# mmammel8/kmer_id

Hardware: AMD Instinct MI355X
Metric: paired reads classified/sec on bact10 DB (higher is better)
Workload: dtype u64

## Files before the change

### include/kmer_id_amd.h

```cpp
#ifndef KMER_ID_AMD_H
#define KMER_ID_AMD_H

#include <stddef.h>
#include <stdint.h>

#ifdef __cplusplus
extern "C" {
#endif

typedef enum kid_status {
    KID_OK = 0,
    KID_ERR_ARG = -1,
    KID_ERR_NOMEM = -2,
    KID_ERR_HIP = -3,
    KID_ERR_TABLE_FULL = -4,
    KID_ERR_TREE = -5,
    KID_ERR_NO_DEVICE = -6,
    KID_ERR_TARGET = -7,
    KID_ERR_IO = -8,
    KID_ERR_FORMAT = -9,
    KID_ERR_STATE = -10
} kid_status;

#define KID_FLAG_U_IS_T 1u
// ... 92 lines not shown
int kid_db_read_hits_time(kid_db *db, double *device_ms, uint64_t *calls, uint64_t *reads);

typedef struct kid_support {
    uint32_t final, confident, n_kmers, n_hits , s_final ,
        s_confident ;
} kid_support;
int kid_db_read_support(kid_db *db, const uint8_t *bases, const uint64_t *offsets, const int32_t *start, const int32_t *stop,
                        uint64_t n_reads, uint32_t min_hits, uint32_t min_permille, kid_support *out, kid_sample *tally);
int kid_db_read_support_fastq(kid_db *db, const uint8_t *text, uint64_t text_nbytes, const kid_fastq_rec *recs, uint64_t n_reads,
                              uint32_t min_hits, uint32_t min_permille, kid_support *out, kid_sample *tally);
int kid_db_support_from_hits_device(kid_db *db, const void *d_hit_offsets, const void *d_hits, const void *d_n_kmers, uint64_t n_reads,
                                    uint32_t min_hits, uint32_t min_permille, void *d_out, void *stream);
int kid_db_read_support_time(kid_db *db, double *device_ms, uint64_t *calls, uint64_t *reads);

#define KID_SEGMENT_MAX_OVERLAP 1024u
typedef struct kid_segment {
    uint32_t pos, n_pos, final, confident, n_kmers, n_hits, s_final, s_confident;
} kid_segment;
int kid_db_read_segments(kid_db *db, const uint8_t *bases, const uint64_t *offsets, const int32_t *start, const int32_t *stop,
                         uint64_t n_reads, uint32_t seg_len, uint32_t seg_step, uint32_t min_hits, uint32_t min_permille,
                         uint64_t *seg_offsets, kid_segment *segments, uint64_t cap, uint64_t *n_segments);
int kid_db_read_segments_fastq(kid_db *db, const uint8_t *text, uint64_t text_nbytes, const kid_fastq_rec *recs, uint64_t n_reads,
                               uint32_t seg_len, uint32_t seg_step, uint32_t min_hits, uint32_t min_permille, uint64_t *seg_offsets,
                               kid_segment *segments, uint64_t cap, uint64_t *n_segments);
int kid_db_read_segments_device(kid_db *db, const void *d_bases, uint64_t bases_nbytes, const void *d_offsets, const void *d_start,
                                const void *d_stop, uint64_t n_reads, uint32_t seg_len, uint32_t seg_step, uint32_t min_hits,
                                uint32_t min_permille, void *d_hits, uint64_t hits_cap, void *d_seg_offsets, void *d_segments,
                                uint64_t seg_cap, void *d_n_hits, void *d_n_segments, void *stream);
int kid_db_read_segments_time(kid_db *db, double *device_ms, uint64_t *calls, uint64_t *reads);

int kid_sample_end(kid_sample *s, int64_t *gcount, int64_t *ucount);
int kid_sample_end_merged(kid_sample **samples, int n, int64_t *gcount, int64_t *ucount);
int kid_sample_stats(kid_sample *s, uint64_t out[4]);

int kid_sample_set_timing(kid_sample *s, int enabled);
int kid_sample_kernel_time(kid_sample *s, double *total_ms, uint64_t *launches);
int kid_sample_kernel_time_device(kid_sample *s, double *total_ms, uint64_t *launches);

int kid_sample_seen_bytes(const kid_sample *s, uint64_t *nbytes);
int kid_sample_seen_export(kid_sample *s, uint64_t byte_off, uint64_t nbytes, void *dst, int dst_on_device);
int kid_sample_seen_or(kid_sample *s, uint64_t byte_off, uint64_t nbytes, const void *src, int src_on_device);
int kid_sample_gcount(kid_sample *s, int64_t *gcount);
int kid_sample_ucount_range(kid_sample *s, uint64_t bit_begin, uint64_t bit_end, int64_t *ucount);

int kid_sample_depth_export(kid_sample *s, uint64_t entry_begin, uint64_t n, void *dst, int dst_on_device);
int kid_sample_depth_add(kid_sample *s, uint64_t entry_begin, uint64_t n, const void *src, int src_on_device);
int kid_sample_depth_spectrum(kid_sample *s, uint32_t bins, uint64_t *spectrum, uint64_t *ksum, uint32_t *dmax);
int kid_sample_depth_spectrum_merged(kid_sample **samples, int n, uint32_t bins, uint64_t *spectrum, uint64_t *ksum, uint32_t *dmax);

typedef struct kid_builder kid_builder;
typedef struct kid_build_cand {
    uint64_t key;
    int64_t gpos;
    int32_t target;
    uint16_t count;
    uint8_t strand_r;
    uint8_t flags;
} kid_build_cand;
int kid_device_mem_info(int device, uint64_t *free_bytes, uint64_t *total_bytes);
int kid_builder_create(int device, int log2_cells, const int32_t *parent, int32_t ntar, uint64_t batch_bases, kid_builder **out);
void kid_builder_destroy(kid_builder *b);
int kid_builder_add(kid_builder *b, const uint8_t *text, uint64_t len, int32_t target);
int kid_builder_remove(kid_builder *b, const uint8_t *text, uint64_t len);
int kid_builder_set_minct(kid_builder *b, const int32_t *minct, int32_t n);
int kid_builder_claim(kid_builder *b, const uint8_t *text, uint64_t len, int64_t gpos_base, kid_build_cand *out, uint64_t cap,
                      uint64_t *n_out);
// ... 11 lines not shown
```

### kmer_id_amd/_lib.py

```python
import ctypes as C
import os

from . import _build

c_u8p = C.POINTER(C.c_uint8)
c_u32p = C.POINTER(C.c_uint32)
c_i32p = C.POINTER(C.c_int32)
c_u64p = C.POINTER(C.c_uint64)
c_i64p = C.POINTER(C.c_int64)
c_void_pp = C.POINTER(C.c_void_p)


class KidDbInfo(C.Structure):
    _fields_ = [
        ("ntar", C.c_int32), ("k", C.c_int32), ("log2_slots", C.c_int32), ("max_probes", C.c_int32),
        ("flags", C.c_uint32), ("device", C.c_int32), ("tree_depth", C.c_int32), ("host_built", C.c_int32),
        ("geometry", C.c_int32), ("reserved_", C.c_int32),
        ("n_entries", C.c_uint64), ("n_occupied", C.c_uint64), ("table_bytes", C.c_uint64),
    ]


PROTOTYPES = {
    "kid_strerror": (C.c_char_p, [C.c_int]),
    "kid_last_error": (C.c_char_p, []),
# ... 23 lines not shown
    "kid_classify_batch_device": (C.c_int, [C.c_void_p, C.c_void_p, C.c_uint64, C.c_void_p, C.c_void_p, C.c_void_p, C.c_uint64,
                                            C.c_void_p, C.c_void_p]),
    "kid_classify_fixed_device": (C.c_int, [C.c_void_p, C.c_void_p, C.c_uint32, C.c_uint64, C.c_void_p, C.c_void_p]),
    "kid_trim_batch": (C.c_int, [C.c_void_p, C.c_void_p, C.c_void_p, C.c_uint64, C.c_void_p, C.c_void_p, C.c_void_p]),
    "kid_db_set_option": (C.c_int, [C.c_void_p, C.c_int, C.c_int]),
    "kid_sample_masked_bases": (C.c_int, [C.c_void_p, c_u64p]),
    "kid_mask_batch": (C.c_int, [C.c_void_p, C.c_void_p, C.c_void_p, C.c_void_p, C.c_uint64, C.c_int, C.c_void_p, c_u64p]),
    "kid_mask_batch_device": (C.c_int, [C.c_void_p, C.c_void_p, C.c_void_p, C.c_void_p, C.c_uint64, C.c_int, C.c_void_p, C.c_void_p]),
    "kid_db_read_hits": (C.c_int, [C.c_void_p, C.c_void_p, C.c_void_p, C.c_void_p, C.c_void_p, C.c_uint64, C.c_void_p, C.c_void_p,
                                   C.c_void_p, C.c_uint64, c_u64p]),
    "kid_db_read_hits_fastq": (C.c_int, [C.c_void_p, C.c_void_p, C.c_uint64, C.c_void_p, C.c_uint64, C.c_void_p, C.c_void_p,
                                         C.c_void_p, C.c_uint64, c_u64p]),
    "kid_db_read_hits_device": (C.c_int, [C.c_void_p, C.c_void_p, C.c_uint64, C.c_void_p, C.c_void_p, C.c_void_p, C.c_uint64,
                                          C.c_void_p, C.c_void_p, C.c_void_p, C.c_uint64, C.c_void_p, C.c_void_p]),
    "kid_db_read_hits_time": (C.c_int, [C.c_void_p, C.POINTER(C.c_double), c_u64p, c_u64p]),
    "kid_db_read_support": (C.c_int, [C.c_void_p, C.c_void_p, C.c_void_p, C.c_void_p, C.c_void_p, C.c_uint64, C.c_uint32, C.c_uint32,
                                      C.c_void_p, C.c_void_p]),
    "kid_db_read_support_fastq": (C.c_int, [C.c_void_p, C.c_void_p, C.c_uint64, C.c_void_p, C.c_uint64, C.c_uint32, C.c_uint32,
                                            C.c_void_p, C.c_void_p]),
    "kid_db_support_from_hits_device": (C.c_int, [C.c_void_p, C.c_void_p, C.c_void_p, C.c_void_p, C.c_uint64, C.c_uint32, C.c_uint32,
                                                  C.c_void_p, C.c_void_p]),
    "kid_db_read_support_time": (C.c_int, [C.c_void_p, C.POINTER(C.c_double), c_u64p, c_u64p]),
    "kid_db_read_segments": (C.c_int, [C.c_void_p, C.c_void_p, C.c_void_p, C.c_void_p, C.c_void_p, C.c_uint64, C.c_uint32, C.c_uint32,
                                       C.c_uint32, C.c_uint32, C.c_void_p, C.c_void_p, C.c_uint64, c_u64p]),
    "kid_db_read_segments_fastq": (C.c_int, [C.c_void_p, C.c_void_p, C.c_uint64, C.c_void_p, C.c_uint64, C.c_uint32, C.c_uint32,
                                             C.c_uint32, C.c_uint32, C.c_void_p, C.c_void_p, C.c_uint64, c_u64p]),
    "kid_db_read_segments_device": (C.c_int, [C.c_void_p, C.c_void_p, C.c_uint64, C.c_void_p, C.c_void_p, C.c_void_p, C.c_uint64,
                                              C.c_uint32, C.c_uint32, C.c_uint32, C.c_uint32, C.c_void_p, C.c_uint64, C.c_void_p,
                                              C.c_void_p, C.c_uint64, C.c_void_p, C.c_void_p, C.c_void_p]),
    "kid_db_read_segments_time": (C.c_int, [C.c_void_p, C.POINTER(C.c_double), c_u64p, c_u64p]),
    "kid_sample_end": (C.c_int, [C.c_void_p, C.c_void_p, C.c_void_p]),
    "kid_sample_end_merged": (C.c_int, [c_void_pp, C.c_int, C.c_void_p, C.c_void_p]),
    "kid_sample_stats": (C.c_int, [C.c_void_p, C.c_void_p]),
    "kid_sample_set_timing": (C.c_int, [C.c_void_p, C.c_int]),
    "kid_sample_kernel_time": (C.c_int, [C.c_void_p, C.POINTER(C.c_double), c_u64p]),
    "kid_sample_kernel_time_device": (C.c_int, [C.c_void_p, C.POINTER(C.c_double), c_u64p]),
    "kid_sample_seen_bytes": (C.c_int, [C.c_void_p, c_u64p]),
    "kid_sample_seen_export": (C.c_int, [C.c_void_p, C.c_uint64, C.c_uint64, C.c_void_p, C.c_int]),
    "kid_sample_seen_or": (C.c_int, [C.c_void_p, C.c_uint64, C.c_uint64, C.c_void_p, C.c_int]),
    "kid_sample_gcount": (C.c_int, [C.c_void_p, C.c_void_p]),
    "kid_sample_ucount_range": (C.c_int, [C.c_void_p, C.c_uint64, C.c_uint64, C.c_void_p]),
    "kid_sample_depth_export": (C.c_int, [C.c_void_p, C.c_uint64, C.c_uint64, C.c_void_p, C.c_int]),
    "kid_sample_depth_add": (C.c_int, [C.c_void_p, C.c_uint64, C.c_uint64, C.c_void_p, C.c_int]),
    "kid_sample_depth_spectrum": (C.c_int, [C.c_void_p, C.c_uint32, C.c_void_p, C.c_void_p, C.c_void_p]),
    "kid_sample_depth_spectrum_merged": (C.c_int, [c_void_pp, C.c_int, C.c_uint32, C.c_void_p, C.c_void_p, C.c_void_p]),
    "kid_synth_db_keys_host": (C.c_int, [C.c_uint64, C.c_int, C.c_void_p, C.c_int32, C.c_uint64, C.c_uint64, C.c_void_p,
                                         C.c_void_p]),
    "kid_synth_db_keys_device": (C.c_int, [C.c_uint64, C.c_int, C.c_void_p, C.c_int32, C.c_uint64, C.c_uint64, C.c_void_p,
                                           C.c_void_p, C.c_int]),
    "kid_synth_reads_host": (C.c_int, [C.c_uint64, C.c_uint64, C.c_int, C.c_void_p, C.c_void_p, C.c_int32, C.c_uint64,
                                       C.c_uint64, C.c_uint32, C.c_void_p]),
    "kid_synth_reads_device": (C.c_int, [C.c_uint64, C.c_uint64, C.c_int, C.c_void_p, C.c_void_p, C.c_int32, C.c_uint64,
                                         C.c_uint64, C.c_uint32, C.c_void_p, C.c_int]),
    "kid_sample_kernel_variants": (C.c_int, [C.c_void_p, c_u64p]),
    "kid_bench_gather": (C.c_int, [C.c_void_p, C.c_uint64, C.c_int, C.c_int, C.POINTER(C.c_float), c_u64p]),
    "kid_dev_alloc": (C.c_int, [C.c_int, C.c_uint64, c_void_pp]),
    "kid_dev_free": (C.c_int, [C.c_int, C.c_void_p]),
    "kid_dev_upload": (C.c_int, [C.c_int, C.c_void_p, C.c_void_p, C.c_uint64]),
    "kid_dev_download": (C.c_int, [C.c_int, C.c_void_p, C.c_void_p, C.c_uint64]),
    "kid_dev_sync": (C.c_int, [C.c_int]),
    "kid_device_mem_info": (C.c_int, [C.c_int, c_u64p, c_u64p]),
    "kid_builder_create": (C.c_int, [C.c_int, C.c_int, C.c_void_p, C.c_int32, C.c_uint64, c_void_pp]),
    "kid_builder_destroy": (None, [C.c_void_p]),
    "kid_builder_add": (C.c_int, [C.c_void_p, C.c_void_p, C.c_uint64, C.c_int32]),
    "kid_builder_remove": (C.c_int, [C.c_void_p, C.c_void_p, C.c_uint64]),
    "kid_builder_set_minct": (C.c_int, [C.c_void_p, C.c_void_p, C.c_int32]),
# ... 64 lines not shown
```

### kmer_id_amd/api.py

```python
import ctypes as C

import numpy as np

from . import _lib
from ._lib import KidDbInfo, check


def _ptr(a):
    return a.ctypes.data_as(C.c_void_p) if a is not None else None


def _as(a, dtype):
    if a is None:
        return None
    a = np.ascontiguousarray(a, dtype=dtype)
    return a


def _offsets_batch(bases, offsets, start, stop):
    offsets = _as(offsets, np.uint64)
    return _as(bases, np.uint8), offsets, _as(start, np.int32), _as(stop, np.int32), offsets.size - 1


def _fastq_block(text, recs):
# ... 351 lines not shown
    def wait(self, ticket):
        check(self._lib.kid_classify_wait(self._h, ticket))

    def classify_device(self, d_bases, bases_nbytes, d_offsets, n_reads, d_start=0, d_stop=0, d_out=0, stream=0):
        check(self._lib.kid_classify_batch_device(self._h, C.c_void_p(d_bases), bases_nbytes, C.c_void_p(d_offsets),
                                                  C.c_void_p(d_start or None), C.c_void_p(d_stop or None), n_reads,
                                                  C.c_void_p(d_out or None), C.c_void_p(stream or None)))

    def classify_fixed_device(self, d_bases, read_len, n_reads, d_out=0, stream=0):
        check(self._lib.kid_classify_fixed_device(self._h, C.c_void_p(d_bases), read_len, n_reads,
                                                  C.c_void_p(d_out or None), C.c_void_p(stream or None)))

    def end(self):
        g = np.empty(self.ntar, np.int64)
        u = np.empty(self.ntar, np.int64)
        check(self._lib.kid_sample_end(self._h, _ptr(g), _ptr(u)))
        return g, u

    def gcount(self):
        g = np.empty(self.ntar, np.int64)
        check(self._lib.kid_sample_gcount(self._h, _ptr(g)))
        return g

    def ucount_range(self, slot_begin, slot_end):
        u = np.empty(self.ntar, np.int64)
        check(self._lib.kid_sample_ucount_range(self._h, slot_begin, slot_end, _ptr(u)))
        return u

    def stats(self):
        out = np.zeros(4, np.uint64)
        check(self._lib.kid_sample_stats(self._h, _ptr(out)))
        return {"reads": int(out[0]), "lookups": int(out[1]), "probes": int(out[2]), "hits": int(out[3])}

    def set_timing(self, enabled=True):
        check(self._lib.kid_sample_set_timing(self._h, 1 if enabled else 0))

    def kernel_time(self):
        ms, n = C.c_double(0), C.c_uint64(0)
        check(self._lib.kid_sample_kernel_time(self._h, C.byref(ms), C.byref(n)))
        return ms.value, n.value

    def kernel_time_device(self):
        ms, n = C.c_double(0), C.c_uint64(0)
        check(self._lib.kid_sample_kernel_time_device(self._h, C.byref(ms), C.byref(n)))
        return ms.value, n.value

    def kernel_variants(self):
        m = C.c_uint64(0)
        check(self._lib.kid_sample_kernel_variants(self._h, C.byref(m)))
        return {(b >> 3 & 1, b >> 2 & 1, b >> 1 & 1, 30 if b & 1 else 0, b >> 4) for b in range(64) if m.value >> b & 1}

    def seen_bytes(self):
        n = C.c_uint64(0)
        check(self._lib.kid_sample_seen_bytes(self._h, C.byref(n)))
        return n.value

    def seen_export(self, byte_off, nbytes, dst_ptr=None, on_device=False):
        if dst_ptr is None:
            buf = np.empty(nbytes, np.uint8)
            check(self._lib.kid_sample_seen_export(self._h, byte_off, nbytes, _ptr(buf), 0))
            return buf
        check(self._lib.kid_sample_seen_export(self._h, byte_off, nbytes, C.c_void_p(dst_ptr), 1 if on_device else 0))
        return None

    def seen_or(self, byte_off, src, nbytes=None, on_device=False):
        if isinstance(src, np.ndarray):
# ... 32 lines not shown
```

### kmer_id_amd/csrc/kid_api.hip

```cpp
#include <hip/hip_runtime.h>
#include <memory>
#include <stdint.h>
#include <string.h>
#include <type_traits>
#include <utility>
#include <vector>

#include "../../include/kmer_id_amd.h"
#include "kid_kernels.hip.h"
#include "kid_build.hip.h"
#include "kid_tile.hip.h"
#include "kid_long.hip.h"
#include "kid_hits.hip.h"
#include "kid_support.hip.h"
#include "kid_segments.hip.h"
#include "kid_mask.hip.h"
#include "kid_depth.hip.h"
#include "kid_api_core.h"
#include "kid_api_db.h"
#include "kid_api_mask.h"
#include "kid_api_hits.h"
#include "kid_api_builder.h"
#include "kid_api_bench.h"

// ... 11 lines not shown
    std::vector<std::pair<KidEvent, KidEvent>> timed;
    uint64_t timed_batches = 0;
    uint32_t batch_seq = 0;
    struct Scratch {
        KidDevBuf desc;
        KidDevBuf long_list;
        KidDevBuf long_plan;
        KidDevBuf rare;
        KidEvent ev_prep;
        KidEvent ev_used;
        hipStream_t used_stream = nullptr;
        bool used_recorded = false;
        bool used = false;
    };
    static const int NSET = 3;
    Scratch sets[NSET];
    uint32_t next_set = 0;
    bool inputs_ready = false;
    int min_base_quality = 0;
    KidDevBuf masked;
    int64_t long_kmers = 65536;
    KidDevBuf rare_fixed;
    struct { uint32_t *out_final = nullptr; uint64_t read0 = 0; uint32_t fixed_len = 0; int32_t fixed_nk = 0; bool valid = false; } fixed_held;
    uint64_t dev_clock_batches = 0;
    KidDevBuf seen_log, seen_log_tail, seen_sorted, log_counts, log_bin_total;
    uint32_t seen_log_cap = 0, log_nbins = 0;
    KidMappedHost log_host_total;
    bool log_dirty = false;
    bool log_off = false;
    uint32_t passes_done = 0;
    uint32_t launches_since_apply = 0;
    uint64_t reads_since_apply = 0;
    double log_entries_per_read = 4.0;
    uint64_t reads_of_last_pass = 0;
    KidDevBuf long_hits, long_tiles;
    bool ended = false;
    uint64_t reads_submitted = 0;
    uint64_t kernel_variants = 0;
    hipStream_t last_stream = nullptr;
    bool has_last_stream = false;
    KidEvent order_ev;
    struct Slot {
        KidDevBuf bases;
        KidDevBuf offsets, start, stop, out;
        KidDevBuf recs;
        KidEvent ev_h2d, ev_done, ev_out;
        std::vector<uint64_t> rel;
        uint64_t ticket = 0;
        bool busy = false;
    };
    static const int NSLOT = 3;
    Slot slots[NSLOT];
    uint64_t next_ticket = 1;

    unsigned long long *stats_p() const { return stats.as<unsigned long long>(); }
    volatile unsigned long long *log_rate() const { return static_cast<volatile unsigned long long *>(log_host_total.p); }
    volatile unsigned int *log_off_flag() const { return reinterpret_cast<volatile unsigned int *>(static_cast<char *>(log_host_total.p) + 8); }
};

extern "C" void kid_sample_destroy(kid_sample *s)
{
    if (!s) return;
    if (s->db) hipSetDevice(s->db->device);
    hipDeviceSynchronize();
    delete s;
}

static int kid_seenlog_point(kid_sample *s, hipStream_t stream);
extern "C" int kid_sample_reset(kid_sample *s)
{
    if (!s) return kid_fail(KID_ERR_ARG, "null sample");
    int rc = kid_use_device(s->db->device);
    if (rc != KID_OK) return rc;
    KID_HIP(hipDeviceSynchronize());
    const size_t nt = (size_t)s->db->info.ntar;
    KID_HIP(hipMemset(s->gcount.p, 0, nt * 8));
    KID_HIP(hipMemset(s->ucount.p, 0, nt * 8));
    KID_HIP(hipMemset(s->stats.p, 0, 256));
    KID_HIP(hipMemset(s->masked.p, 0, 8));
    {
        const unsigned long long never = ~0ull;
        KID_HIP(hipMemcpy(s->stats_p() + 30, &never, 8, hipMemcpyHostToDevice));
    }
    s->dev_clock_batches = 0;
    s->reads_submitted = 0;
    s->ended = false;
    s->kernel_variants = 0;
    if (s->seen_log_tail.p) KID_HIP(hipMemset(s->seen_log_tail.p, 0, KID_LOG_SHARDS * 64));
    if (s->seen_log.p) {
        int rc = kid_seenlog_point(s, nullptr);
        if (rc != KID_OK) return rc;
        *s->log_off_flag() = 0;
        *s->log_rate() = 0;
        s->log_off = false;
        s->passes_done = 0;
        s->log_entries_per_read = 4.0;
    }
    s->log_dirty = false;
    s->launches_since_apply = 0;
    s->reads_since_apply = 0;
    KID_HIP(hipMemset(s->seen.p, 0, s->seen_words * 4));
    if (s->depth.p) KID_HIP(hipMemset(s->depth.p, 0, s->seen_words * 32 * 4));
    KID_HIP(hipDeviceSynchronize());
    return KID_OK;
}

extern "C" int kid_sample_begin(kid_db *db, kid_sample **out)
{
    if (!db || !out) return kid_fail(KID_ERR_ARG, "null argument");
    *out = nullptr;
    int rc = kid_use_device(db->device);
    if (rc != KID_OK) return rc;
    std::unique_ptr<kid_sample, void (*)(kid_sample *)> s(new kid_sample(), kid_sample_destroy);
    s->db = db;
    const size_t nt = (size_t)db->info.ntar;
    s->seen_words = db->seen_bits / 32;
    KID_HIP(s->gcount.alloc(nt * 8));
    KID_HIP(s->ucount.alloc(nt * 8));
    KID_HIP(s->stats.alloc(256));
    KID_HIP(s->masked.alloc(8));
    KID_HIP(s->seen.alloc(s->seen_words * 4));
    KID_HIP(s->stream.create());
    const uint64_t nbins = (db->seen_bits + (1ull << KID_LOG_BIN_BITS) - 1) >> KID_LOG_BIN_BITS;
    if (db->d.minloc && nbins <= 1024) {
        uint64_t total = db->info.n_entries * 2ull;
        if (total < (32ull << 20)) total = 32ull << 20;
        if (total > (128ull << 20)) total = 128ull << 20;
        uint64_t cap = (total / KID_LOG_SHARDS) & ~63ull;
        s->seen_log_cap = (uint32_t)cap;
// ... 3 lines not shown
        KID_HIP(s->seen_log_tail.alloc(KID_LOG_SHARDS * 64));
        KID_HIP(s->log_counts.alloc(nbins * KID_LOG_WGS * 4));
        KID_HIP(s->log_bin_total.alloc(nbins * 4));
        KID_HIP(s->log_host_total.alloc(64, hipHostMallocMapped));
        memset(s->log_host_total.p, 0, 64);
    }
    const KidRareArgs ra{s->gcount.as<unsigned long long>(), s->stats_p(), db->d.line_mask, 0u, 0ull, 0ull, 0, 0u, db->d.rows,
                         s->seen.as<uint32_t>(), nullptr, nullptr, s->seen_log.as<uint32_t>(), s->seen_log_tail.as<uint32_t>(),
                         s->seen_log_cap, 0u};
    for (kid_sample::Scratch &sc : s->sets) {
        KID_HIP(sc.rare.alloc(sizeof(ra)));
        KID_HIP(hipMemcpy(sc.rare.p, &ra, sizeof(ra), hipMemcpyHostToDevice));
        KID_HIP(sc.ev_prep.create(hipEventDisableTiming));
        KID_HIP(sc.ev_used.create(hipEventDisableTiming));
    }
    KID_HIP(s->rare_fixed.alloc(sizeof(ra)));
    KID_HIP(hipMemcpy(s->rare_fixed.p, &ra, sizeof(ra), hipMemcpyHostToDevice));
    rc = kid_sample_reset(s.get());
    if (rc != KID_OK) return rc;
    *out = s.release();
    return KID_OK;
}

static int kid_seenlog_apply(kid_sample *s, hipStream_t stream)
{
    if (!s->seen_log.p || !s->log_dirty) return KID_OK;
    void *dev_total = nullptr;
    KID_HIP(hipHostGetDevicePointer(&dev_total, s->log_host_total.p, 0));
    const KidLogArgs a{s->seen_log.as<uint32_t>(), s->seen_log_tail.as<uint32_t>(), s->seen_log_cap, s->log_nbins,
                       s->log_counts.as<uint32_t>(), s->log_bin_total.as<uint32_t>(), s->seen_sorted.as<uint32_t>(),
                       s->seen.as<uint32_t>(), s->seen_words, (unsigned long long *)dev_total, s->reads_since_apply,
                       {s->sets[0].rare.as<KidRareArgs>(), s->sets[1].rare.as<KidRareArgs>(), s->sets[2].rare.as<KidRareArgs>(),
                        s->rare_fixed.as<KidRareArgs>()},
                       (unsigned int *)((char *)dev_total + 8)};
    static_assert(kid_sample::NSET == 3, "KidLogArgs::blocks");
    const uint32_t nb = s->log_nbins;
    hipLaunchKernelGGL(kid_seenlog_count_kernel, dim3(KID_LOG_WGS), dim3(256), nb * 4, stream, a);
    hipLaunchKernelGGL(kid_seenlog_scan_kernel, dim3(nb), dim3(KID_LOG_WGS), 0, stream, a);
    hipLaunchKernelGGL(kid_seenlog_scatter_kernel, dim3(KID_LOG_WGS), dim3(256), (4 * nb + 1 + KID_LOG_TILE) * 4, stream, a);
    hipLaunchKernelGGL(kid_seenlog_apply_kernel, dim3(nb), dim3(1024), ((1u << (KID_LOG_BIN_BITS - 5)) + nb + 1) * 4, stream, a);
    KID_HIP(hipMemsetAsync(s->seen_log_tail.p, 0, KID_LOG_SHARDS * 64, stream));
    KID_HIP(hipGetLastError());
    s->reads_of_last_pass = s->reads_since_apply;
    s->log_dirty = false;
    s->launches_since_apply = 0;
    s->reads_since_apply = 0;
    s->passes_done++;
    return KID_OK;
}
static int kid_seenlog_flush(kid_sample *s)
{
    if (!s->seen_log.p || !s->log_dirty) return KID_OK;
    KID_HIP(hipDeviceSynchronize());
    return kid_seenlog_apply(s, s->stream.s);
}
static int kid_seenlog_point(kid_sample *s, hipStream_t stream)
{
    KidRareArgs *blocks[kid_sample::NSET + 1];
    int nb = 0;
    for (kid_sample::Scratch &sc : s->sets) blocks[nb++] = sc.rare.as<KidRareArgs>();
    blocks[nb++] = s->rare_fixed.as<KidRareArgs>();
    for (int i = 0; i < nb; i++)
        if (blocks[i]) KID_HIP(hipMemcpyAsync(&blocks[i]->seen_log, &s->seen_log.p, sizeof(uint32_t *), hipMemcpyHostToDevice, stream));
    return KID_OK;
}
static int kid_seenlog_pace(kid_sample *s, uint64_t n_reads, hipStream_t stream)
{
    if (!s->seen_log.p || s->log_off) return KID_OK;
    if (*s->log_off_flag()) {
        s->log_off = true;
        return KID_OK;
    }
    const unsigned long long rate = *s->log_rate();
    if (rate >> 63) {
        const double r = (double)(rate & ~(1ull << 63)) / 1024.0;
        s->log_entries_per_read = r > 0.01 ? r * 1.1 : 0.011;
    }
    const double room = 0.5 * (double)s->seen_log_cap * KID_LOG_SHARDS;
    if (s->log_dirty && ((double)(s->reads_since_apply + n_reads) * s->log_entries_per_read > room || s->launches_since_apply >= 256)) {
        int rc = kid_seenlog_apply(s, stream);
        if (rc != KID_OK) return rc;
    }
    s->reads_since_apply += n_reads;
    s->launches_since_apply++;
    s->log_dirty = true;
    return KID_OK;
}

static int kid_sample_order_behind(kid_sample *s, hipStream_t stream)
{
    if (s->has_last_stream && s->last_stream != stream) {
        if (!s->order_ev.e) KID_HIP(s->order_ev.create(hipEventDisableTiming));
        KID_HIP(hipEventRecord(s->order_ev.e, s->last_stream));
        KID_HIP(hipStreamWaitEvent(stream, s->order_ev.e, 0));
    }
    s->last_stream = stream;
    s->has_last_stream = true;
    return KID_OK;
}

template <class F> static inline void kid_lift(bool v, F &&f)
{
    if (v) f(std::true_type{});
    else f(std::false_type{});
}

static int kid_launch_classify(kid_sample *s, const KidBatch &b, uint64_t bases_nbytes, hipStream_t stream, int64_t max_kmers,
                               hipStream_t prep_stream, bool long_records = false, const KidFastqRec *fastq = nullptr)
{
    kid_db *db = s->db;
    if (b.n == 0) return KID_OK;
    if (b.n > 0x7FFFFFFFull) return kid_fail(KID_ERR_ARG, "at most 2^31-1 reads per batch");
    if (bases_nbytes >> 48) return kid_fail(KID_ERR_ARG, "a batch of 2^48 bytes or more");
    const bool fixed = b.offsets == nullptr && !fastq;
    const uint32_t long_cut = (long_records && !fastq && s->long_kmers > 0 && s->long_kmers < 0xFFFFFFFFll &&
                               bases_nbytes > (uint64_t)s->long_kmers) ? (uint32_t)s->long_kmers : 0u;
    if (long_cut) max_kmers = -1;
    {
        int rc = kid_sample_order_behind(s, stream);
        if (rc == KID_OK) rc = kid_seenlog_pace(s, b.n, stream);
        if (rc != KID_OK) return rc;
    }
    unsigned long long *const gcount = s->gcount.as<unsigned long long>(), *const stats = s->stats_p();
    uint32_t *const seen = s->seen.as<uint32_t>();
    kid_sample::Scratch *scp = nullptr;
    KidRareArgs *rare = s->rare_fixed.as<KidRareArgs>();
    KidReadDesc *desc = nullptr;
    if (!fixed) {
        kid_sample::Scratch &sc = s->sets[s->next_set++ % kid_sample::NSET];
        scp = &sc;
        rare = sc.rare.as<KidRareArgs>();
        if (b.n * sizeof(KidReadDesc) > sc.desc.cap) KID_HIP(hipDeviceSynchronize());
        KID_HIP(sc.desc.ensure(b.n * sizeof(KidReadDesc), b.n * sizeof(KidReadDesc)));
        desc = sc.desc.as<KidReadDesc>();
        if (long_cut) {
            if (!sc.long_plan.p) {
                KID_HIP(sc.long_list.alloc(sizeof(KidLongList)));
                KID_HIP(hipMemset(sc.long_list.p, 0, 16));
                KID_HIP(sc.long_plan.alloc(sizeof(KidLongPlan)));
            }
            const uint64_t want = bases_nbytes < (128ull << 20) ? bases_nbytes : (128ull << 20);
            if (want * 4 > s->long_hits.cap) {
                KID_HIP(hipDeviceSynchronize());
                const uint64_t cap = want + want / 4;
                s->long_hits.reset();
                s->long_tiles.reset();
                KID_HIP(s->long_tiles.ensure(cap / 256 + KID_LONG_MAX + 16, cap / 256 + KID_LONG_MAX + 16));
                KID_HIP(s->long_hits.ensure(want * 4, cap * 4));
            }
        }
        if (sc.used && sc.used_stream != prep_stream) {
            if (sc.used_recorded || hipEventRecord(sc.ev_used.e, sc.used_stream) == hipSuccess) KID_HIP(hipStreamWaitEvent(prep_stream, sc.ev_used.e, 0));
            else {
// ... 2 lines not shown
            }
        }
        const bool fuse_rebase = prep_stream == stream;
        if (fastq)
            hipLaunchKernelGGL(kid_prepare_fastq_kernel, dim3(kid_grid_for(b.n, 256, db->num_cu * 8)), dim3(256), 0, prep_stream, b.bases,
                               fastq, b.n, db->info.k, desc, const_cast<int32_t *>(b.start), const_cast<int32_t *>(b.stop),
                               b.out_final, stats, gcount, rare, ++s->batch_seq, fuse_rebase ? 1 : 0);
        else
            hipLaunchKernelGGL(kid_prepare_kernel, dim3(kid_grid_for(b.n, 256, db->num_cu * 8)), dim3(256), 0, prep_stream, b, db->info.k,
                               desc, stats, rare, ++s->batch_seq, long_cut, sc.long_list.as<KidLongList>(), fuse_rebase ? 1 : 0);
        if (prep_stream != stream) {
            KID_HIP(hipEventRecord(sc.ev_prep.e, prep_stream));
            KID_HIP(hipStreamWaitEvent(stream, sc.ev_prep.e, 0));
        }
        if (long_cut)
            hipLaunchKernelGGL(kid_long_plan_kernel, dim3(1), dim3(64), 0, stream, sc.long_list.as<KidLongList>(), sc.long_plan.as<KidLongPlan>(),
                               desc, rare, s->batch_seq, (uint64_t)s->long_hits.cap / 4, (uint64_t)s->long_tiles.cap - 16);
    }
    const int block = 512, wpb = block / 64;
    const uint32_t ntar = (uint32_t)db->info.ntar;
    const bool ml = db->d.minloc != 0;
    const int grid = kid_grid_for(b.n, wpb, db->num_cu * 16);
    const uint32_t hist_words32 = (ntar + 3u) & ~3u, hist_words16 = ((ntar + 1u) / 2u + 3u) & ~3u;
    const uint32_t hist_words = ml ? hist_words16 : hist_words32;
    const uint32_t wave_words = ml ? KID_GEN_ML_LDS_WORDS : KID_WAVE_LDS_WORDS;
    const bool hist = (hist_words + wpb * wave_words) * 4u + 32u <= 40u * 1024u;
    const bool hist_pair = (hist_words16 + wpb * KID_PAIR_LDS_WORDS) * 4u + 32u <= 40u * 1024u;
    uint64_t span = b.n;
    if (ml && (hist || hist_pair)) {
        const uint64_t per_wg = (uint64_t)(65535u - 2u * (uint32_t)wpb - 64u * (uint32_t)wpb) * (KID_TAPER + 1u) / (2u * KID_TAPER);
        const uint64_t cap = (uint64_t)grid * ((grid & 1) ? per_wg / 2 : per_wg);
        if (span > cap) span = cap;
    }
    KidSampleDev sd{gcount, seen, stats};
    const bool rows = db->d.rows != nullptr, k30 = db->info.k == 30;
    const int32_t fixed_nk = fixed ? (int32_t)(max_kmers > 0 ? max_kmers : 0) : 0;
    const bool want_pair = ml && (max_kmers < 0 || max_kmers <= 2 * 64);
    const bool want_duo = ml && (max_kmers < 0 || (max_kmers > 2 * 64 && max_kmers <= 4 * 64));
    const bool want_general = !ml || max_kmers < 0 || max_kmers > 4 * 64;
    KidEvent ev0, ev1;
    if (s->timing) {
        KID_HIP(ev0.create());
        KID_HIP(ev1.create());
        KID_HIP(hipEventRecord(ev0.e, stream));
    }
    for (uint64_t r0 = 0; r0 < b.n; r0 += span) {
        const uint64_t cnt = b.n - r0 < span ? b.n - r0 : span;
        KidInput pk{b.bases, fixed ? nullptr : desc + r0, b.out_final ? b.out_final + r0 : nullptr, cnt};
        if (fixed) {
            auto &h = s->fixed_held;
            if (!h.valid || h.out_final != pk.out_final || h.read0 != r0 || h.fixed_len != b.fixed_len || h.fixed_nk != fixed_nk) {
                hipLaunchKernelGGL(kid_rebase_kernel, dim3(1), dim3(64), 0, stream, rare, (const KidReadDesc *)nullptr, pk.out_final,
                                   (unsigned long long)r0, b.fixed_len, fixed_nk, (1ull << 32) | (unsigned long long)fixed_nk);
                h.valid = true; h.out_final = pk.out_final; h.read0 = r0; h.fixed_len = b.fixed_len; h.fixed_nk = fixed_nk;
            }
        } else if (r0 != 0 || prep_stream != stream) {
            hipLaunchKernelGGL(kid_rebase_kernel, dim3(1), dim3(64), 0, stream, rare, pk.desc, pk.out_final, 0ull, 0u, 0, 0ull);
        }
        auto launch = [&](auto pk_mode, bool h) {
            constexpr int PK = decltype(pk_mode)::value;
            kid_lift(rows, [&](auto R) { kid_lift(h, [&](auto H) { kid_lift(ml, [&](auto M) { kid_lift(k30, [&](auto K30) {
                if constexpr (PK == 0 || decltype(M)::value) {
                    constexpr bool r = decltype(R)::value, hh = decltype(H)::value, m = decltype(M)::value;
                    constexpr int KF = decltype(K30)::value ? 30 : 0;
                    const uint32_t hw = hh ? (PK ? hist_words16 : hist_words) : 0u;
                    s->kernel_variants |= 1ull << (PK * 16 | r << 3 | hh << 2 | m << 1 | (KF == 30));
                    hipLaunchKernelGGL((kid_classify_kernel<2, r, hh, m, KF, PK>), dim3(grid), dim3(block),
                                       (hw + (size_t)wpb * (PK ? KID_PAIR_LDS_WORDS : wave_words)) * 4 + 32, stream, db->d, pk, sd, hw,
                                       pk.desc, rare);
                }
            }); }); }); });
        };
        if (want_pair) launch(std::integral_constant<int, 1>{}, hist_pair);
        if (want_duo) launch(std::integral_constant<int, 2>{}, hist_pair);
        if (want_general) launch(std::integral_constant<int, 0>{}, hist);
    }
    if (long_cut) {
        hipLaunchKernelGGL(kid_long_hits_kernel, dim3((unsigned)db->num_cu * 8u), dim3(256), 0, stream, db->d, b.bases,
                           scp->long_plan.as<KidLongPlan>(), s->long_hits.as<uint32_t>(), s->long_tiles.as<uint8_t>(), seen, stats);
        hipLaunchKernelGGL(kid_long_fold_kernel, dim3(KID_LONG_MAX), dim3(256), 0, stream, db->d, scp->long_plan.as<KidLongPlan>(),
// ... 15 lines not shown
    s->reads_submitted += b.n;
    return KID_OK;
}

static int kid_depth_set_option(kid_sample *s, int value);
extern "C" int kid_sample_set_option(kid_sample *s, int option, int value)
{
    if (!s) return kid_fail(KID_ERR_ARG, "null sample");
    switch (option) {
    case KID_OPT_INPUTS_READY: s->inputs_ready = value != 0; return KID_OK;
    case KID_OPT_LONG_RECORD_KMERS:
        if (value < 0) return kid_fail(KID_ERR_ARG, "KID_OPT_LONG_RECORD_KMERS: negative threshold");
        s->long_kmers = value;
        return KID_OK;
    case KID_OPT_MIN_BASE_QUALITY: {
        int rc = kid_mask_check_q(value);
        if (rc == KID_OK) s->min_base_quality = value;
        return rc;
    }
    case KID_OPT_ENTRY_DEPTH: return kid_depth_set_option(s, value);
    default: return kid_fail(KID_ERR_ARG, "unknown option %d", option);
    }
}

static int kid_prep_stream_for(kid_sample *s, hipStream_t stream, hipStream_t *out)
{
    *out = stream;
    if (!s->inputs_ready) return KID_OK;
    if (!s->prep_stream.s) KID_HIP(s->prep_stream.create(hipStreamNonBlocking));
    *out = s->prep_stream.s;
    return KID_OK;
}

extern "C" int kid_sample_kernel_variants(kid_sample *s, uint64_t *mask)
{
    if (!s || !mask) return kid_fail(KID_ERR_ARG, "null argument");
    *mask = s->kernel_variants;
    return KID_OK;
}

extern "C" int kid_sample_set_timing(kid_sample *s, int enabled)
{
    if (!s) return kid_fail(KID_ERR_ARG, "null sample");
    s->timing = enabled != 0;
    return KID_OK;
}

extern "C" int kid_sample_kernel_time(kid_sample *s, double *total_ms, uint64_t *launches)
{
    if (!s || !total_ms || !launches) return kid_fail(KID_ERR_ARG, "null argument");
    int rc = kid_use_device(s->db->device);
    if (rc != KID_OK) return rc;
    KID_HIP(hipDeviceSynchronize());
    double sum = 0;
    for (auto &ev : s->timed) {
        float ms = 0;
        KID_HIP(hipEventElapsedTime(&ms, ev.first.e, ev.second.e));
        sum += ms;
    }
    *total_ms = sum;
    *launches = s->timed_batches;
    s->timed.clear();
    s->timed_batches = 0;
    return KID_OK;
}

// ... 411 lines not shown
```

### kmer_id_amd/csrc/kid_kernels.hip.h

```cpp
#pragma once
#include <hip/hip_runtime.h>
#include <stdint.h>
#include <type_traits>
#include "kid_common.h"

#define KID_WAVE 64
#define KID_TOMBSTONE_HI 0xFFFFFFFFu
#define KID_SEG_KMERS 960
#define KID_WAVE_LDS_WORDS 104
#define KID_CQ_CAP 192
#define KID_CQ_FLUSH 64
#define KID_PAIR_LDS_WORDS (4 + 3 * KID_CQ_CAP + KID_CQ_CAP / 4 + 64 + 128)
#define KID_TAPER 6u
#define KID_EARLY_MAX 4u
#define KID_EARLY_QN 32u
#define KID_GEN_ML_LDS_WORDS (104 + 3 * KID_CQ_CAP + KID_CQ_CAP / 4 + 64)
#define KID_CLASSIFY_OCC 8
#define KID_CLASSIFY_OCC_DUO_ROWS 4

typedef uint32_t kid_u4 __attribute__((ext_vector_type(4)));
typedef uint32_t kid_u2 __attribute__((ext_vector_type(2)));

__device__ __forceinline__ void kid_store_u32_nowait(uint32_t *p, uint32_t v)
{
// ... 1485 lines not shown
            const uint32_t h = (uint32_t)kid_fmix64(key) & slot_mask;
            uint32_t rp = 0, i = 0;
            for (;;) {
                const uint32_t idx = (h + rp) & slot_mask;
                rp += ++i;
                const uint32_t *c = reinterpret_cast<const uint32_t *>(table + idx);
                const uint32_t ord = c[3];
                if (ord == 0) break;
                if (c[0] == (uint32_t)key && c[1] == (uint32_t)(key >> 32)) {
                    if (ord == (uint32_t)e + 1u) my_idx = idx;
                    min_ord = ord < min_ord ? ord : min_ord;
                    copies++;
                }
            }
        }
        if (copies > 1 && min_ord != (uint32_t)e + 1u) reinterpret_cast<uint32_t *>(table + my_idx)[1] = KID_TOMBSTONE_HI;
    }
}

struct KidLogArgs {
    const uint32_t *log;
    const uint32_t *tail;
    uint32_t cap;
    uint32_t nbins;
    uint32_t *counts;
    uint32_t *bin_total;
    uint32_t *sorted;
    uint32_t *seen;
    uint64_t seen_words;
    unsigned long long *host_total;
    unsigned long long reads;
    KidRareArgs *blocks[4];
    unsigned int *off_flag;
};
__device__ __forceinline__ void kid_log_share(const KidLogArgs &a, uint32_t &begin, uint32_t &end)
{
    const uint32_t per = KID_LOG_WGS / KID_LOG_SHARDS, sh = blockIdx.x / per, c = blockIdx.x % per;
    const uint32_t t = a.tail[sh * 16u], filled = t < a.cap ? t : a.cap;
    const uint32_t len = ((filled + per - 1u) / per + 63u) & ~63u;
    begin = sh * a.cap + (c * len < filled ? c * len : filled);
    end = sh * a.cap + ((c + 1u) * len < filled ? (c + 1u) * len : filled);
}
template <class F>
__device__ __forceinline__ void kid_log_for_each(const uint32_t *log, uint32_t b0, uint32_t b1, F &&f)
{
    const uint32_t n4 = (b1 - b0) >> 2;
    const uint4 *p = reinterpret_cast<const uint4 *>(log + b0);
    for (uint32_t i = threadIdx.x; i < n4; i += blockDim.x) {
        const uint4 v = p[i];
        if (v.x != KID_LOG_NONE) f(v.x);
        if (v.y != KID_LOG_NONE) f(v.y);
        if (v.z != KID_LOG_NONE) f(v.z);
        if (v.w != KID_LOG_NONE) f(v.w);
    }
    for (uint32_t i = b0 + (n4 << 2) + threadIdx.x; i < b1; i += blockDim.x) {
        const uint32_t e = log[i];
        if (e != KID_LOG_NONE) f(e);
    }
}
__global__ __launch_bounds__(256) void kid_seenlog_count_kernel(const KidLogArgs a)
{
    extern __shared__ uint32_t kid_lh[];
    for (uint32_t i = threadIdx.x; i < a.nbins; i += blockDim.x) kid_lh[i] = 0;
    __syncthreads();
    uint32_t b0, b1;
    kid_log_share(a, b0, b1);
// ... 48 lines not shown
        for (uint32_t i0 = 0; i0 < a.nbins; i0 += 64u) {
            const uint32_t i = i0 + threadIdx.x;
            const uint32_t v = i < a.nbins ? a.bin_total[i] : 0u, x = kid_wave_incscan(v);
            if (i < a.nbins) bases[i] = run + x - v;
            run += (uint32_t)__shfl((int)x, 63);
        }
        if (threadIdx.x == 0) bases[a.nbins] = run;
    }
    __syncthreads();
    return bases[a.nbins];
}
__device__ __forceinline__ uint32_t kid_block_exscan(const uint32_t *v, uint32_t *out, const uint32_t n, uint32_t *wave_tot )
{
    const uint32_t i0 = 4u * threadIdx.x;
    uint32_t x[4];
#pragma unroll
    for (int j = 0; j < 4; j++) x[j] = i0 + j < n ? v[i0 + j] : 0u;
    kid_block_exscan4(x, wave_tot);
#pragma unroll
    for (int j = 0; j < 4; j++) if (i0 + j < n) out[i0 + j] = x[j];
    const uint32_t total = wave_tot[0] + wave_tot[1] + wave_tot[2] + wave_tot[3];
    __syncthreads();
    return total;
}
#define KID_LOG_TILE 4096u
__global__ __launch_bounds__(256) void kid_seenlog_scatter_kernel(const KidLogArgs a)
{
    extern __shared__ uint32_t kid_lh[];
    const uint32_t nb = a.nbins;
    uint32_t *bases = kid_lh, *next = bases + nb + 1u, *hist = next + nb, *toff = hist + nb, *stage = toff + nb;
    __shared__ uint32_t wave_tot[5];
    kid_log_bin_bases(a, bases);
    if (blockIdx.x == 0 && threadIdx.x == 0) {
        unsigned long long asked = 0;
        for (uint32_t i = 0; i < KID_LOG_SHARDS; i++) asked += a.tail[i * 16u];
        if (a.host_total && a.reads) *a.host_total = ((asked << 10) / a.reads) | (1ull << 63);
        if (a.reads && asked > 8ull * a.reads) {
            for (int i = 0; i < 4; i++)
                if (a.blocks[i]) a.blocks[i]->seen_log = nullptr;
            if (a.off_flag) *a.off_flag = 1u;
        }
    }
    for (uint32_t i = threadIdx.x; i < nb; i += blockDim.x) next[i] = bases[i] + a.counts[i * KID_LOG_WGS + blockIdx.x];
    uint32_t b0, b1;
    kid_log_share(a, b0, b1);
    for (uint32_t t0 = b0; t0 < b1; t0 += KID_LOG_TILE) {
        const uint32_t n = b1 - t0 < KID_LOG_TILE ? b1 - t0 : KID_LOG_TILE;
        for (uint32_t i = threadIdx.x; i < nb; i += blockDim.x) hist[i] = 0;
        __syncthreads();
        uint32_t e[KID_LOG_TILE / 256u], r[KID_LOG_TILE / 256u];
#pragma unroll
        for (uint32_t j = 0; j < KID_LOG_TILE / 256u; j++) {
            const uint32_t i = j * 256u + threadIdx.x;
            e[j] = i < n ? a.log[t0 + i] : KID_LOG_NONE;
        }
#pragma unroll
        for (uint32_t j = 0; j < KID_LOG_TILE / 256u; j++)
            r[j] = e[j] != KID_LOG_NONE ? atomicAdd(&hist[e[j] >> KID_LOG_BIN_BITS], 1u) : 0u;
        __syncthreads();
        const uint32_t tile_n = kid_block_exscan(hist, toff, nb, wave_tot);
#pragma unroll
        for (uint32_t j = 0; j < KID_LOG_TILE / 256u; j++)
            if (e[j] != KID_LOG_NONE) stage[toff[e[j] >> KID_LOG_BIN_BITS] + r[j]] = e[j];
        __syncthreads();
        for (uint32_t p = threadIdx.x; p < tile_n; p += blockDim.x) {
            const uint32_t v = stage[p], bin = v >> KID_LOG_BIN_BITS;
            a.sorted[next[bin] + (p - toff[bin])] = v;
        }
// ... 71 lines not shown
```

Measured before the change: 1.156 billion.

## Split classify launches to fit seen-log capacity and carry measured log rate across resets

The seen-log pacing call moves from before the launch to inside the per-chunk loop. The launch span is now capped by how many reads the log room can hold at the current estimated entries-per-read rate, so one large batch no longer overflows the shard logs and forces the log off. The measured rate is kept across sample resets instead of falling back to the default. A small diagnostic API reporting passes, placed entries and overflowed regions is also added. The cost is more, smaller launches and more frequent apply passes whenever the log rate is high.

```diff
diff --git a/include/kmer_id_amd.h b/include/kmer_id_amd.h
--- a/include/kmer_id_amd.h
+++ b/include/kmer_id_amd.h
@@ -148,6 +148,7 @@
 int kid_sample_end(kid_sample *s, int64_t *gcount, int64_t *ucount);
 int kid_sample_end_merged(kid_sample **samples, int n, int64_t *gcount, int64_t *ucount);
 int kid_sample_stats(kid_sample *s, uint64_t out[4]);
+int kid_sample_log_info(kid_sample *s, uint64_t out[4]);
 
 int kid_sample_set_timing(kid_sample *s, int enabled);
 int kid_sample_kernel_time(kid_sample *s, double *total_ms, uint64_t *launches);
diff --git a/kmer_id_amd/_lib.py b/kmer_id_amd/_lib.py
--- a/kmer_id_amd/_lib.py
+++ b/kmer_id_amd/_lib.py
@@ -79,6 +79,7 @@
     "kid_sample_end": (C.c_int, [C.c_void_p, C.c_void_p, C.c_void_p]),
     "kid_sample_end_merged": (C.c_int, [c_void_pp, C.c_int, C.c_void_p, C.c_void_p]),
     "kid_sample_stats": (C.c_int, [C.c_void_p, C.c_void_p]),
+    "kid_sample_log_info": (C.c_int, [C.c_void_p, C.c_void_p]),
     "kid_sample_set_timing": (C.c_int, [C.c_void_p, C.c_int]),
     "kid_sample_kernel_time": (C.c_int, [C.c_void_p, C.POINTER(C.c_double), c_u64p]),
     "kid_sample_kernel_time_device": (C.c_int, [C.c_void_p, C.POINTER(C.c_double), c_u64p]),
diff --git a/kmer_id_amd/api.py b/kmer_id_amd/api.py
--- a/kmer_id_amd/api.py
+++ b/kmer_id_amd/api.py
@@ -407,6 +407,11 @@
         check(self._lib.kid_sample_stats(self._h, _ptr(out)))
         return {"reads": int(out[0]), "lookups": int(out[1]), "probes": int(out[2]), "hits": int(out[3])}
 
+    def log_info(self):
+        out = np.zeros(4, np.uint64)
+        check(self._lib.kid_sample_log_info(self._h, _ptr(out)))
+        return {"passes": int(out[0]), "places": int(out[1]), "overflowed_regions": int(out[2]), "off": bool(out[3])}
+
     def set_timing(self, enabled=True):
         check(self._lib.kid_sample_set_timing(self._h, 1 if enabled else 0))
 
diff --git a/kmer_id_amd/csrc/kid_api.hip b/kmer_id_amd/csrc/kid_api.hip
--- a/kmer_id_amd/csrc/kid_api.hip
+++ b/kmer_id_amd/csrc/kid_api.hip
@@ -67,6 +67,7 @@
     uint32_t launches_since_apply = 0;
     uint64_t reads_since_apply = 0;
     double log_entries_per_read = 4.0;
+    bool log_rate_known = false;
     uint64_t reads_of_last_pass = 0;
     KidDevBuf long_hits, long_tiles;
     bool ended = false;
@@ -91,6 +92,8 @@
     unsigned long long *stats_p() const { return stats.as<unsigned long long>(); }
     volatile unsigned long long *log_rate() const { return static_cast<volatile unsigned long long *>(log_host_total.p); }
     volatile unsigned int *log_off_flag() const { return reinterpret_cast<volatile unsigned int *>(static_cast<char *>(log_host_total.p) + 8); }
+    volatile unsigned long long *log_applied() const { return log_rate() + 2; }
+    double log_room() const { return 0.5 * (double)seen_log_cap * KID_LOG_SHARDS; }
 };
 
 extern "C" void kid_sample_destroy(kid_sample *s)
@@ -102,6 +105,7 @@
 }
 
 static int kid_seenlog_point(kid_sample *s, hipStream_t stream);
+static void kid_seenlog_listen(kid_sample *s);
 extern "C" int kid_sample_reset(kid_sample *s)
 {
     if (!s) return kid_fail(KID_ERR_ARG, "null sample");
@@ -125,11 +129,14 @@
     if (s->seen_log.p) {
         int rc = kid_seenlog_point(s, nullptr);
         if (rc != KID_OK) return rc;
+        if (!s->log_off && !*s->log_off_flag()) kid_seenlog_listen(s);
         *s->log_off_flag() = 0;
         *s->log_rate() = 0;
+        s->log_applied()[0] = 0;
+        s->log_applied()[1] = 0;
         s->log_off = false;
         s->passes_done = 0;
-        s->log_entries_per_read = 4.0;
+        if (!s->log_rate_known) s->log_entries_per_read = 4.0;
     }
     s->log_dirty = false;
     s->launches_since_apply = 0;
@@ -199,7 +206,7 @@
                        s->seen.as<uint32_t>(), s->seen_words, (unsigned long long *)dev_total, s->reads_since_apply,
                        {s->sets[0].rare.as<KidRareArgs>(), s->sets[1].rare.as<KidRareArgs>(), s->sets[2].rare.as<KidRareArgs>(),
                         s->rare_fixed.as<KidRareArgs>()},
-                       (unsigned int *)((char *)dev_total + 8)};
+                       (unsigned int *)((char *)dev_total + 8), (unsigned long long *)dev_total + 2};
     static_assert(kid_sample::NSET == 3, "KidLogArgs::blocks");
     const uint32_t nb = s->log_nbins;
     hipLaunchKernelGGL(kid_seenlog_count_kernel, dim3(KID_LOG_WGS), dim3(256), nb * 4, stream, a);
@@ -231,19 +238,36 @@
         if (blocks[i]) KID_HIP(hipMemcpyAsync(&blocks[i]->seen_log, &s->seen_log.p, sizeof(uint32_t *), hipMemcpyHostToDevice, stream));
     return KID_OK;
 }
-static int kid_seenlog_pace(kid_sample *s, uint64_t n_reads, hipStream_t stream)
-{
-    if (!s->seen_log.p || s->log_off) return KID_OK;
+static void kid_seenlog_listen(kid_sample *s)
+{
+    if (!s->seen_log.p || s->log_off) return;
     if (*s->log_off_flag()) {
         s->log_off = true;
-        return KID_OK;
+        return;
     }
     const unsigned long long rate = *s->log_rate();
     if (rate >> 63) {
         const double r = (double)(rate & ~(1ull << 63)) / 1024.0;
         s->log_entries_per_read = r > 0.01 ? r * 1.1 : 0.011;
-    }
-    const double room = 0.5 * (double)s->seen_log_cap * KID_LOG_SHARDS;
+        s->log_rate_known = true;
+    }
+}
+#define KID_LOG_MAX_RATE 8.0
+static uint64_t kid_seenlog_launch_reads(kid_sample *s, uint64_t n_reads)
+{
+    kid_seenlog_listen(s);
+    if (!s->seen_log.p || s->log_off) return n_reads;
+    const double room = s->log_room();
+    if (!s->log_rate_known && (double)n_reads * KID_LOG_MAX_RATE > room && s->log_entries_per_read < KID_LOG_MAX_RATE)
+        s->log_entries_per_read = KID_LOG_MAX_RATE;
+    const double fit = room / s->log_entries_per_read;
+    return fit >= (double)n_reads ? n_reads : fit < 65536.0 ? 65536ull : (uint64_t)fit;
+}
+static int kid_seenlog_pace(kid_sample *s, uint64_t n_reads, hipStream_t stream)
+{
+    kid_seenlog_listen(s);
+    if (!s->seen_log.p || s->log_off) return KID_OK;
+    const double room = s->log_room();
     if (s->log_dirty && ((double)(s->reads_since_apply + n_reads) * s->log_entries_per_read > room || s->launches_since_apply >= 256)) {
         int rc = kid_seenlog_apply(s, stream);
         if (rc != KID_OK) return rc;
@@ -285,7 +309,6 @@
     if (long_cut) max_kmers = -1;
     {
         int rc = kid_sample_order_behind(s, stream);
-        if (rc == KID_OK) rc = kid_seenlog_pace(s, b.n, stream);
         if (rc != KID_OK) return rc;
     }
     unsigned long long *const gcount = s->gcount.as<unsigned long long>(), *const stats = s->stats_p();
@@ -354,6 +377,10 @@
         const uint64_t cap = (uint64_t)grid * ((grid & 1) ? per_wg / 2 : per_wg);
         if (span > cap) span = cap;
     }
+    if (ml) {
+        const uint64_t fit = kid_seenlog_launch_reads(s, b.n);
+        if (span > fit) span = fit;
+    }
     KidSampleDev sd{gcount, seen, stats};
     const bool rows = db->d.rows != nullptr, k30 = db->info.k == 30;
     const int32_t fixed_nk = fixed ? (int32_t)(max_kmers > 0 ? max_kmers : 0) : 0;
@@ -361,6 +388,10 @@
     const bool want_duo = ml && (max_kmers < 0 || (max_kmers > 2 * 64 && max_kmers <= 4 * 64));
     const bool want_general = !ml || max_kmers < 0 || max_kmers > 4 * 64;
     KidEvent ev0, ev1;
+    {
+        int rc = kid_seenlog_pace(s, b.n < span ? b.n : span, stream);
+        if (rc != KID_OK) return rc;
+    }
     if (s->timing) {
         KID_HIP(ev0.create());
         KID_HIP(ev1.create());
@@ -368,6 +399,10 @@
     }
     for (uint64_t r0 = 0; r0 < b.n; r0 += span) {
         const uint64_t cnt = b.n - r0 < span ? b.n - r0 : span;
+        if (r0 != 0) {
+            int rc = kid_seenlog_pace(s, cnt, stream);
+            if (rc != KID_OK) return rc;
+        }
         KidInput pk{b.bases, fixed ? nullptr : desc + r0, b.out_final ? b.out_final + r0 : nullptr, cnt};
         if (fixed) {
             auto &h = s->fixed_held;
@@ -449,6 +484,22 @@
     return KID_OK;
 }
 
+extern "C" int kid_sample_log_info(kid_sample *s, uint64_t out[4])
+{
+    if (!s || !out) return kid_fail(KID_ERR_ARG, "null argument");
+    out[0] = out[1] = out[2] = 0;
+    out[3] = 1;
+    if (!s->seen_log.p) return KID_OK;
+    int rc = kid_use_device(s->db->device);
+    if (rc != KID_OK) return rc;
+    KID_HIP(hipDeviceSynchronize());
+    out[0] = s->passes_done;
+    out[1] = s->log_applied()[0];
+    out[2] = s->log_applied()[1];
+    out[3] = (s->log_off || *s->log_off_flag()) ? 1 : 0;
+    return KID_OK;
+}
+
 extern "C" int kid_sample_kernel_variants(kid_sample *s, uint64_t *mask)
 {
     if (!s || !mask) return kid_fail(KID_ERR_ARG, "null argument");
diff --git a/kmer_id_amd/csrc/kid_kernels.hip.h b/kmer_id_amd/csrc/kid_kernels.hip.h
--- a/kmer_id_amd/csrc/kid_kernels.hip.h
+++ b/kmer_id_amd/csrc/kid_kernels.hip.h
@@ -1541,6 +1541,7 @@
     unsigned long long reads;
     KidRareArgs *blocks[4];
     unsigned int *off_flag;
+    unsigned long long *applied;
 };
 __device__ __forceinline__ void kid_log_share(const KidLogArgs &a, uint32_t &begin, uint32_t &end)
 {
@@ -1655,8 +1656,14 @@
     __shared__ uint32_t wave_tot[5];
     kid_log_bin_bases(a, bases);
     if (blockIdx.x == 0 && threadIdx.x == 0) {
-        unsigned long long asked = 0;
-        for (uint32_t i = 0; i < KID_LOG_SHARDS; i++) asked += a.tail[i * 16u];
+        unsigned long long asked = 0, held = 0, over = 0;
+        for (uint32_t i = 0; i < KID_LOG_SHARDS; i++) {
+            const uint32_t t = a.tail[i * 16u];
+            asked += t;
+            held += t < a.cap ? t : a.cap;
+            over += t > a.cap ? 1u : 0u;
+        }
+        if (a.applied) { a.applied[0] += held; a.applied[1] += over; }
         if (a.host_total && a.reads) *a.host_total = ((asked << 10) / a.reads) | (1ull << 63);
         if (a.reads && asked > 8ull * a.reads) {
             for (int i = 0; i < 4; i++)
```

Result: no change. 1.153 billion (-0.2%).
